# Zachary-Luk/3D-Denoising-Diffusion-Model

Measured on AMD Instinct MI355X. Metric: denoised 64³ volumes/sec @250 DDPM steps, 1/2/4/8 MI355X; PSNR vs ref, higher is better.
Workload: dtype f32 (conv products: 3x f16-split MFMA, f32 accumulate)

## Files before the change

3d-denoising-diffusion-model_amd/csrc/api.hip:

```cpp
#include <hip/hip_runtime.h>
#include <stdarg.h>
#include <stdio.h>
#include <string.h>
#include "conv3d_params.h"
#include "ddpm3d.h"
#include "ops.h"

static thread_local char g_err[512] = "";

static int fail(int code, const char* fmt, ...) {
    va_list ap;
    va_start(ap, fmt);
    vsnprintf(g_err, sizeof(g_err), fmt, ap);
    va_end(ap);
    return code;
}
static int launched(hipError_t e, const char* what) {
    if (e == hipSuccess) return DDPM3D_OK;
    return fail(DDPM3D_ELAUNCH, "%s: %s", what, hipGetErrorString(e));
}
static bool aligned16(const void* p) { return (reinterpret_cast<uintptr_t>(p) & 15) == 0; }

extern "C" {

// ... 22 lines not shown
    if (!aligned16(out)) return fail(DDPM3D_EINVAL, "pack_conv_weight: w_packed must be 16-byte aligned");
    if (prec_wz(precision) && !wz_layer_ok(Cout, Cin, ksize))
        return fail(DDPM3D_ENOSUP, "pack_conv_weight: the Winograd-D form needs ksize 3, Cout %% 128 == 0, "
                                   "Cin %% 16 == 0 (got Cout=%d Cin=%d k=%d)", Cout, Cin, ksize);
    return launched(ddpm3d_launch_pack(w, Cout, Cin, ksize, precision, out, (hipStream_t)stream),
                    "pack_conv_weight");
}

size_t ddpm3d_packed_up_phase_bytes(int Cout, int Cin) {
    if (Cout <= 0 || Cin <= 0 || !wz_layer_ok(Cout, Cin, 3)) return 0;
    return ddpm3d_up_phase_bytes(Cout, Cin);
}

int ddpm3d_pack_up_phase_weight(const float* w, int Cout, int Cin, void* out, void* stream) {
    if (!w || !out || Cout <= 0 || Cin <= 0)
        return fail(DDPM3D_EINVAL, "pack_up_phase_weight: bad arguments (Cout=%d Cin=%d)", Cout, Cin);
    if (!aligned16(out)) return fail(DDPM3D_EINVAL, "pack_up_phase_weight: w_packed must be 16-byte aligned");
    if (!wz_layer_ok(Cout, Cin, 3))
        return fail(DDPM3D_ENOSUP, "pack_up_phase_weight: needs Cout %% 128 == 0, Cin %% 16 == 0 (got Cout=%d Cin=%d)",
                    Cout, Cin);
    return launched(ddpm3d_launch_pack_up_phase(w, Cout, Cin, out, (hipStream_t)stream), "pack_up_phase_weight");
}

int ddpm3d_conv_stats_rows(int N, int D, int H, int W, int Cin, int Cout, int ksize, int precision) {
    if (N <= 0 || D <= 0 || H <= 0 || W <= 0 || Cin <= 0 || Cout <= 0 || !prec_ok(precision)) return 0;
    return ddpm3d_conv_cfg(N, D, H, W, Cin, Cout, ksize, precision).stats_rows;
}

size_t ddpm3d_conv_workspace_bytes(int N, int D, int H, int W, int Cin, int Cout, int ksize, int precision) {
    if (N <= 0 || D <= 0 || H <= 0 || W <= 0 || Cin <= 0 || Cout <= 0 || !prec_ok(precision)) return 0;
    return ddpm3d_conv_cfg(N, D, H, W, Cin, Cout, ksize, precision).workspace_bytes;
}

enum { ROUTE_GENERAL = 0, ROUTE_SKINNY = 1, ROUTE_PW = 2 };
static int conv_prepare(const ddpm3d_conv_desc* d, ConvK& k, ConvCfg& c, int& route, bool for_launch) {
    if (!d) return fail(DDPM3D_EINVAL, "conv3d: null descriptor");
    if (d->N <= 0 || d->D <= 0 || d->H <= 0 || d->W <= 0 || d->Cout <= 0 || d->Cin <= 0)
        return fail(DDPM3D_EINVAL, "conv3d: non-positive shape N=%d D=%d H=%d W=%d Cin=%d Cout=%d", d->N, d->D,
                    d->H, d->W, d->Cin, d->Cout);
    if (d->ksize != 1 && d->ksize != 3) return fail(DDPM3D_EINVAL, "conv3d: ksize %d (1 or 3)", d->ksize);
    if (!prec_ok(d->precision)) return fail(DDPM3D_ENOSUP, "conv3d: precision mode %d not implemented", d->precision);
    if (d->C0 + d->C1 != d->Cin) return fail(DDPM3D_EINVAL, "conv3d: C0+C1 != Cin");
    if (for_launch && (!d->src0 || !d->w_packed || !d->bias || !d->out)) return fail(DDPM3D_EINVAL, "conv3d: null buffer");
    if (d->in_mode == DDPM3D_IN_PLANAR2) {
        if (d->Cin != 2 || d->C0 != 1 || d->C1 != 1 || (for_launch && !d->src1) || d->aff_a)
            return fail(DDPM3D_EINVAL, "conv3d: planar2 input needs C0=C1=1, two planes, no affine");
    } else {
        if (d->in_mode < 0 || d->in_mode > DDPM3D_IN_STRIDE2) return fail(DDPM3D_EINVAL, "conv3d: in_mode %d", d->in_mode);
        if (d->in_mode == DDPM3D_IN_STRIDE2 && d->ksize != 3)
            return fail(DDPM3D_EINVAL, "conv3d: the strided input mode is the 3x3x3 Downsample conv's");
        if (d->Cin % DDPM3D_CONV_CK) return fail(DDPM3D_EINVAL, "conv3d: Cin=%d not a multiple of %d", d->Cin, DDPM3D_CONV_CK);
        if (d->C1 > 0 && (d->C0 % DDPM3D_CONV_CK || (for_launch && !d->src1)))
            return fail(DDPM3D_EINVAL, "conv3d: concat needs C0 %% %d == 0 and src1", DDPM3D_CONV_CK);
        if (!aligned16(d->src0) || (d->src1 && !aligned16(d->src1)))
            return fail(DDPM3D_EINVAL, "conv3d: sources must be 16-byte aligned");
        if (d->in_mode == DDPM3D_IN_UP && ((d->H | d->W) & 1))
            return fail(DDPM3D_EINVAL, "conv3d: upsampled input needs even H, W (got %d, %d)", d->H, d->W);
    }
    if ((d->aff_a == nullptr) != (d->aff_b == nullptr)) return fail(DDPM3D_EINVAL, "conv3d: aff_a/aff_b must come together");
    if (d->aff_a && (!aligned16(d->aff_a) || !aligned16(d->aff_b)))
        return fail(DDPM3D_EINVAL, "conv3d: affine tables must be 16-byte aligned");
    if (!aligned16(d->w_packed)) return fail(DDPM3D_EINVAL, "conv3d: w_packed must be 16-byte aligned");
    if (d->res_mode < 0 || d->res_mode > 3 || (d->res_mode != DDPM3D_RES_NONE && !d->res))
        return fail(DDPM3D_EINVAL, "conv3d: residual mode %d without / with bad buffer", d->res_mode);
    if (d->res_mode == DDPM3D_RES_UP && ((d->H | d->W) & 1))
        return fail(DDPM3D_EINVAL, "conv3d: upsampled residual needs even H, W");
    if (d->bias_stride_n < 0) return fail(DDPM3D_EINVAL, "conv3d: negative bias_stride_n");
    if (d->out_layout != DDPM3D_OUT_NDHWC && d->out_layout != DDPM3D_OUT_NCDHW)
        return fail(DDPM3D_EINVAL, "conv3d: out_layout %d", d->out_layout);

    c = ddpm3d_conv_cfg(d->N, d->D, d->H, d->W, d->Cin, d->Cout, d->ksize, d->precision);
    if (d->kernel_hint & DDPM3D_HINT_SPLITK_MASK) {
        const int s_forced = (d->kernel_hint & DDPM3D_HINT_SPLITK_MASK) >> DDPM3D_HINT_SPLITK_SHIFT;
        const int nch = ddpm3d_cin_pad(d->Cin) / DDPM3D_CONV_CK;
        if (s_forced > nch || (s_forced != c.S && c.WN != 4))
            return fail(DDPM3D_EINVAL, "conv3d: a forced split factor needs Cout > 64 and S <= Cin / 16");
        ddpm3d_conv_cfg_split(c, s_forced, d->N, d->D, d->H, d->W, d->Cout);
    }
    if (prec_wz(d->precision) &&
        !(wz_layer_ok(d->Cout, d->Cin, d->ksize) && c.WN == 4 && c.MT == 4 &&
          (d->in_mode == DDPM3D_IN_SAME || d->in_mode == DDPM3D_IN_UP)))
        return fail(DDPM3D_ENOSUP, "conv3d: the Winograd-D form needs ksize 3, Cout %% 128 == 0 "
                                   "and input mode SAME or UP; use the F16X3 packing for this call");
    if (for_launch && c.S > 1 && (!d->workspace || d->workspace_bytes < c.workspace_bytes || !aligned16(d->workspace)))
        return fail(DDPM3D_EINVAL, "conv3d: this shape is split %d-way over Cin and needs %zu bytes of "
                                   "16-byte aligned workspace (got %zu)", c.S, c.workspace_bytes,
                    d->workspace ? d->workspace_bytes : (size_t)0);
    memset(&k, 0, sizeof(k));
    k.src0 = d->src0; k.src1 = d->src1; k.affA = d->aff_a; k.affB = d->aff_b;
    k.w = (const float*)d->w_packed; k.bias = d->bias; k.res = d->res; k.out = d->out; k.stats = d->stats;
    k.N = d->N; k.D = d->D; k.H = d->H; k.W = d->W; k.Cin = d->Cin; k.Cout = d->Cout;
    k.C0 = d->C0; k.C1 = d->C1;
    k.CinPad = ddpm3d_cin_pad(d->Cin); k.CoutPad = ddpm3d_cout_pad(d->Cout);
    k.in_mode = d->in_mode; k.act = d->act; k.bias_stride_n = d->bias_stride_n;
    k.res_mode = d->res_mode; k.out_layout = d->out_layout;
    k.tilesZ = c.tilesZ; k.tilesY = c.tilesY; k.tilesX = c.tilesX;
    k.stats_rows = c.stats_rows;
    k.reduce_vox = c.reduce_vox;
    k.hint = d->kernel_hint;
    bool phase = false;
    if (d->kernel_hint & DDPM3D_HINT_UP_PHASE) {
        if (d->precision != DDPM3D_PREC_F16X3_WZ || d->in_mode != DDPM3D_IN_UP)
            return fail(DDPM3D_EINVAL, "conv3d: DDPM3D_HINT_UP_PHASE needs precision F16X3_WZ and in_mode UP");
        UpPhaseGeom g;
// ... 29 lines not shown
        const long long vox = (long long)d->N * d->D * Hs * Ws;
        const long long b0 = vox * d->C0 * ((d->io_dtype & DDPM3D_IO_SRC0_BF16) ? 2 : 4);
        const long long b1 = vox * d->C1 * ((d->io_dtype & DDPM3D_IO_SRC1_BF16) ? 2 : 4);
        const size_t wb = phase ? ddpm3d_up_phase_body_bytes(d->Cout, d->Cin)
                                : ddpm3d_packed_bytes(d->Cout, d->Cin, d->ksize, d->precision);
        if (b0 >= 0xFFFFFFF0LL || b1 >= 0xFFFFFFF0LL || wb >= 0xFFFFFFF0ULL)
            return fail(DDPM3D_E2BIG, "conv3d: a source tensor or the weights exceed 4 GiB; split the batch");
        if ((long long)d->D * d->H * d->W * d->Cout * 4 >= 0xFFFFFFF0LL)
            return fail(DDPM3D_E2BIG, "conv3d: one output sample exceeds 4 GiB; tile the volume");
        k.src0_bytes = (unsigned)b0; k.src1_bytes = (unsigned)b1; k.w_bytes = (unsigned)wb;
        k.wstat = (d->kernel_hint & DDPM3D_HINT_WSTAT_ON)    ? 1
                  : (d->kernel_hint & DDPM3D_HINT_WSTAT_OFF) ? 0
                                                             : ((long long)wb > b0 + b1 ? 1 : 0);
    }
    if (phase)
        k.wscale = (const float*)((const char*)k.w + ddpm3d_up_phase_body_bytes(d->Cout, d->Cin));
    else if (c.PREC != DDPM3D_PREC_F32)
        k.wscale = (const float*)((const char*)d->w_packed +
                                  ddpm3d_packed_bytes(d->Cout, d->Cin, d->ksize, d->precision) -
                                  (size_t)ddpm3d_cout_pad(d->Cout) * 4);
    if (d->stats && d->stats_rows != k.stats_rows)
        return fail(DDPM3D_EINVAL, "conv3d: stats_rows=%d, this shape writes %d", d->stats_rows, k.stats_rows);
    if (d->stats && !aligned16(d->stats)) return fail(DDPM3D_EINVAL, "conv3d: stats must be 16-byte aligned");
    if (d->stats && d->out_layout != DDPM3D_OUT_NDHWC)
        return fail(DDPM3D_EINVAL, "conv3d: statistics only with NDHWC output");
    const long long blocks = (long long)k.N * k.tilesZ * k.tilesY * k.tilesX;
    if (blocks > 0x7fffffffLL) return fail(DDPM3D_EINVAL, "conv3d: grid too large");
    if (d->ksize == 3 && d->Cout <= 2 && d->in_mode == DDPM3D_IN_SAME && d->C1 == 0 && !d->stats &&
        d->res_mode == DDPM3D_RES_NONE &&
        ddpm3d_skinny_ok(k.CinPad, d->precision, !(d->io_dtype & DDPM3D_IO_SRC0_BF16) ? 0
                                                  : ((d->io_dtype & DDPM3D_IO_HALF_IS_F16) ? 2 : 1)))
        route = ROUTE_SKINNY;
    else
        route = ddpm3d_pw_ok(k, c, d->ksize) ? ROUTE_PW : ROUTE_GENERAL;
    return DDPM3D_OK;
}

int ddpm3d_conv3d(const ddpm3d_conv_desc* d, void* stream) {
    ConvK k;
    ConvCfg c;
    int route = ROUTE_GENERAL;
    const int ok = conv_prepare(d, k, c, route, true);
    if (ok != DDPM3D_OK) return ok;
    if (route == ROUTE_SKINNY)
        return launched(ddpm3d_launch_conv_skinny(k, d->precision, (hipStream_t)stream), "conv3d (skinny)");
    const int rc = route == ROUTE_PW ? launched(ddpm3d_launch_conv_pw(k, c, (hipStream_t)stream), "conv3d (1x1)")
                                     : launched(ddpm3d_launch_conv(k, c, (hipStream_t)stream), "conv3d");
    if (rc != DDPM3D_OK || c.S == 1) return rc;
    return launched(ddpm3d_launch_splitk_reduce(k, (hipStream_t)stream), "conv3d split-K reduce");
}

int ddpm3d_conv_plan(const ddpm3d_conv_desc* d, int* stats_rows, size_t* workspace_bytes, int* split) {
    ConvK k;
    ConvCfg c;
    int route = ROUTE_GENERAL;
    const int ok = conv_prepare(d, k, c, route, false);
    if (ok != DDPM3D_OK) return ok;
    if (stats_rows) *stats_rows = c.stats_rows;
    if (workspace_bytes) *workspace_bytes = c.workspace_bytes;
    if (split) *split = c.S;
    return DDPM3D_OK;
}

int ddpm3d_conv_kernel_family(const ddpm3d_conv_desc* d, char* name, int name_len) {
    if (!name || name_len <= 0) return fail(DDPM3D_EINVAL, "conv_kernel_family: no buffer");
    ConvK k;
    ConvCfg c;
    int route = ROUTE_GENERAL;
    const int ok = conv_prepare(d, k, c, route, false);
    if (ok != DDPM3D_OK) return ok;
    const int tile = 1 << c.TXL;
    int n;
    if (route == ROUTE_SKINNY) n = snprintf(name, (size_t)name_len, "conv3d_p%d_k3_skinny", d->precision);
    else if (route == ROUTE_PW) n = snprintf(name, (size_t)name_len, "conv1x1_p%d_t%d", d->precision, tile);
    else n = snprintf(name, (size_t)name_len, "conv3d_p%d_k%d_wn%d_t%d", d->precision, d->ksize, c.WN, tile);
    if (n < 0 || n >= name_len) return fail(DDPM3D_EINVAL, "conv_kernel_family: buffer of %d bytes is too short", name_len);
    return DDPM3D_OK;
}

int ddpm3d_gn_finalize(const double* stats0, int C0, int rows0, const double* stats1, int C1, int rows1,
// ... 505 lines not shown
```

3d-denoising-diffusion-model_amd/csrc/conv3d_params.h:

```cpp
#pragma once
#include <hip/hip_runtime.h>
#include <stddef.h>
#include <stdlib.h>
#include "ddpm3d.h"

#define DDPM3D_CONV_CK 16
#define DDPM3D_REDUCE_VOX 16
#define DDPM3D_X3_W_TARGET 8.0f

struct ConvK {
    const float* src0;
    const float* src1;
    const float* affA;
    const float* affB;
    const float* w;
    const float* bias;
    const float* res;
    float* out;
    double* stats;
    float* partial;
    const float* wscale;
    const float* in_bound;
    int in_bound_count, in_bound_stride;
    unsigned w_bytes, src0_bytes, src1_bytes;
    int N, D, H, W, Cin, Cout, C0, C1, CinPad, CoutPad;
    int in_mode, act, bias_stride_n, res_mode, out_layout, stats_rows;
    int tilesX, tilesY, tilesZ;
    int ksplit, chunks_per_split;
    int wstat;
    int reduce_vox;
    int hint;
    int io;
};

struct ConvCfg {
    int PREC;
    int KS;
    int WN;
    int MT;
    int TXL, TYL;
    int S;
    int tilesX, tilesY, tilesZ;
    int stats_rows;
    int reduce_vox;
    size_t workspace_bytes;
};

static inline int ddpm3d_round_up(int v, int m) { return (v + m - 1) / m * m; }
static inline int ddpm3d_cout_pad(int Cout) { return ddpm3d_round_up(Cout, 32); }
static inline int ddpm3d_cin_pad(int Cin) { return ddpm3d_round_up(Cin, DDPM3D_CONV_CK); }

static inline void ddpm3d_conv_cfg_split(ConvCfg& c, int S, int N, int D, int H, int W, int Cout) {
    const long long vox = (long long)D * H * W;
    c.S = S;
    if (S > 1) {
        c.stats_rows = (int)((vox + c.reduce_vox - 1) / c.reduce_vox);
        c.workspace_bytes = (size_t)S * N * vox * Cout * sizeof(float);
    } else {
        c.stats_rows = c.tilesZ * c.tilesY * c.tilesX * (4 / c.WN);
        c.workspace_bytes = 0;
    }
}

static inline ConvCfg ddpm3d_conv_cfg(int N, int D, int H, int W, int Cin, int Cout, int ksize, int prec) {
    ConvCfg c;
    c.PREC = prec;
    const bool one_mfma = prec == DDPM3D_PREC_F16 || prec == DDPM3D_PREC_F16_WZ || prec == DDPM3D_PREC_BF16 ||
                          prec == DDPM3D_PREC_BF16_WZ;
    c.KS = ksize;
    c.WN = Cout > 64 ? 4 : (Cout > 32 ? 2 : 1);
#ifdef DDPM3D_FORCE_T4_3X3
    if (H >= 8 && W >= 8 && ksize != 3) { c.TXL = 3; c.TYL = 3; } else { c.TXL = 2; c.TYL = 2; }
#else
    if (H >= 8 && W >= 8) { c.TXL = 3; c.TYL = 3; } else { c.TXL = 2; c.TYL = 2; }
#endif
    c.MT = c.WN;
    const int TX = 1 << c.TXL, TY = 1 << c.TYL, TZ = (4 / c.WN) * c.MT * 32 / (TX * TY);
    c.tilesX = (W + TX - 1) / TX;
    c.tilesY = (H + TY - 1) / TY;
    c.tilesZ = (D + TZ - 1) / TZ;
    const long long mtiles = (long long)N * c.tilesZ * c.tilesY * c.tilesX;
    const long long blocks = mtiles * ((ddpm3d_cout_pad(Cout) + 32 * c.WN - 1) / (32 * c.WN));
    const int nch = ddpm3d_cin_pad(Cin) / DDPM3D_CONV_CK;
    int best = 1;
    if (ksize == 1 && c.WN == 4) {
        double best_cost = 1e300;
        for (int s = 1; s <= 32 && s <= nch; ++s) {
            const int cps = (nch + s - 1) / s;
            if (s > 1 && cps < 4) break;
            const long long per_cu = (blocks * s + 255) / 256;
            const double cost = (double)per_cu * (0.25 * cps + 6.0) + (s > 1 ? 6.0 : 0.0);
            if (cost < best_cost * 0.9) { best_cost = cost; best = s; }
        }
    }
    if (ksize == 3 && c.WN == 4 && !one_mfma) {
        static const double eff[4] = {1.0, 0.62, 0.78, 0.82};
        double best_cost = 1e300;
        for (int s = 1; s <= 16 && s <= nch; ++s) {
            const int cps = (nch + s - 1) / s;
            if (s > 1 && cps < 2) break;
            const long long per_cu = (blocks * s + 255) / 256;
            const double e = eff[per_cu > 3 ? 3 : (int)per_cu];
            const double cost = (double)per_cu * (cps + (s > 1 ? 0.75 : 0.5)) / e;
            if (cost < best_cost * 0.99) { best_cost = cost; best = s; }
        }
    }
    if (ksize == 3 && c.WN == 4 && one_mfma) {
        static const double eff[4] = {1.0, 0.5, 1.0, 0.9};
        static const int cand[] = {1, 2, 3, 4, 5, 6, 8, 10, 12, 16};
        const double out_mb = (double)N * D * H * W * Cout * 4.0 / 1e6;
        double best_cost = 1e300;
        for (int i = 0; i < 10 && cand[i] <= nch; ++i) {
            const int s = cand[i];
            const int cps = (nch + s - 1) / s;
            if (s > 1 && cps < 2) break;
            const long long per_cu = (blocks * s + 255) / 256;
            const double e = eff[per_cu > 3 ? 3 : (int)per_cu];
            const double cost = (double)per_cu * (cps + (s > 1 ? 3.0 : 0.25)) / e + (s > 1 ? 0.2 * s * out_mb : 0.0);
// ... 32 lines not shown
    const int TZ = 128 / (g.TX * g.TY);
    g.tilesX = (Wl + g.TX - 1) / g.TX;
    g.tilesY = (Hl + g.TY - 1) / g.TY;
    g.tilesZ = (D + TZ - 1) / TZ;
    return 4LL * g.tilesX * g.tilesY * g.tilesZ == (long long)c.tilesX * c.tilesY * c.tilesZ;
}

struct DynLdsOnce { unsigned long long mask[4]; };
static inline hipError_t ddpm3d_allow_dynamic_lds(DynLdsOnce& done, const void* kernel, int bytes) {
    int dev = 0;
    hipError_t e = hipGetDevice(&dev);
    if (e != hipSuccess) return e;
    dev &= 255;
    unsigned long long& w = done.mask[dev >> 6];
    const unsigned long long bit = 1ull << (dev & 63);
    if (__atomic_load_n(&w, __ATOMIC_ACQUIRE) & bit) return hipSuccess;
    e = hipFuncSetAttribute(kernel, hipFuncAttributeMaxDynamicSharedMemorySize, bytes);
    if (e == hipSuccess) __atomic_fetch_or(&w, bit, __ATOMIC_RELEASE);
    return e;
}

hipError_t ddpm3d_launch_conv(const ConvK& k, const ConvCfg& c, hipStream_t st);
hipError_t ddpm3d_launch_splitk_reduce(const ConvK& k, hipStream_t st);
hipError_t ddpm3d_launch_conv_skinny(const ConvK& k, int prec, hipStream_t st);
hipError_t ddpm3d_launch_conv_pw(const ConvK& k, const ConvCfg& c, hipStream_t st);
static inline bool ddpm3d_pw_ok(const ConvK& k, const ConvCfg& c, int ksize) {
    const bool s0 = (k.io & DDPM3D_IO_SRC0_BF16) != 0, s1 = (k.io & DDPM3D_IO_SRC1_BF16) != 0;
    return ksize == 1 && (c.PREC == 1 || c.PREC == 2 || c.PREC == 5) && c.WN == 4 && c.MT == 4 &&
           k.in_mode == DDPM3D_IN_SAME && k.affA == nullptr && k.act == 0 && k.stats == nullptr &&
           k.Cout % 128 == 0 && k.Cin % 32 == 0 && k.C0 % 32 == 0 && (k.C1 == 0 || s0 == s1) &&
           (k.ksplit == 1 || k.chunks_per_split % 2 == 0);
}
bool ddpm3d_skinny_ok(int CinPad, int prec, int src16);

struct GnAcc {
#ifdef DDPM3D_STATS_F64
    double a1, a2;
    __device__ __forceinline__ void init(float) { a1 = 0.0; a2 = 0.0; }
    __device__ __forceinline__ void add(float v) { const double d = (double)v; a1 += d; a2 = __builtin_fma(d, d, a2); }
    __device__ __forceinline__ double sum1(float) const { return a1; }
    __device__ __forceinline__ double sum2(float) const { return a2; }
#else
    float p, s1, s2;
    __device__ __forceinline__ void init(float pivot) { p = pivot; s1 = 0.0f; s2 = 0.0f; }
    __device__ __forceinline__ void add(float v) { const float d = v - p; s1 += d; s2 = __builtin_fmaf(d, d, s2); }
    __device__ __forceinline__ double sum1(float n) const { return (double)n * (double)p + (double)s1; }
    __device__ __forceinline__ double sum2(float n) const {
        const double dp = (double)p;
        return (double)s2 + 2.0 * dp * (double)s1 + (double)n * dp * dp;
    }
#endif
};

__device__ __forceinline__ float ddpm3d_half_to_float(unsigned short h, bool f16) {
    if (f16) return (float)__builtin_bit_cast(_Float16, h);
    return __builtin_bit_cast(float, (unsigned)h << 16);
}
__device__ __forceinline__ float ddpm3d_act_load(const float* base, size_t e, bool b16, bool f16) {
    if (b16) return ddpm3d_half_to_float(reinterpret_cast<const unsigned short*>(base)[e], f16);
    return base[e];
}
__device__ __forceinline__ unsigned short ddpm3d_to_bf16(float v) {
    return __builtin_bit_cast(unsigned short, (__bf16)v);
}
__device__ __forceinline__ unsigned short ddpm3d_to_half(float v, bool f16) {
    if (f16) return __builtin_bit_cast(unsigned short, (_Float16)v);
// ... 30 lines not shown
```

3d-denoising-diffusion-model_amd/guided_diffusion/_hip.py:

```python

import ctypes as C
import os

import torch

_HERE = os.path.dirname(os.path.abspath(__file__))
LIB_PATH = os.environ.get("DDPM3D_LIB") or os.path.normpath(os.path.join(_HERE, "..", "csrc", "libddpm3d.so"))

IN_SAME, IN_POOL, IN_UP, IN_PLANAR2, IN_STRIDE2 = 0, 1, 2, 3, 4
RES_NONE, RES_SAME, RES_POOL, RES_UP = 0, 1, 2, 3
ACT_NONE, ACT_SILU = 0, 1
OUT_NDHWC, OUT_NCDHW = 0, 1
F_LEARN_SIGMA, F_PREDICT_XSTART, F_CLIP = 1, 2, 4
NCOEF = 8
NQCOEF = 4
NSCOEF = 8
S_CX, S_W0, S_W1, S_W2, S_CZ = 0, 1, 2, 3, 4
PREC_F32, PREC_F16X3, PREC_F16, PREC_F16X3_WZ, PREC_F16_WZ, PREC_BF16, PREC_BF16_WZ = 0, 1, 2, 3, 4, 5, 6
PRECISIONS = {"f32": PREC_F32, "f16x3": PREC_F16X3, "f16": PREC_F16, "bf16": PREC_BF16}
WINOGRAD_OF = {PREC_F16X3: PREC_F16X3_WZ, PREC_F16: PREC_F16_WZ, PREC_BF16: PREC_BF16_WZ}
IO_SRC0_BF16, IO_SRC1_BF16, IO_OUT_BF16, IO_RES_BF16 = 1, 2, 4, 8
IO_HALF_IS_F16 = 16
ABI_VERSION = 13
MAX_DRAWS = 64
HINT_WSTAT_OFF, HINT_WSTAT_ON = 0x100, 0x200
HINT_SPLITK_SHIFT = 16
HINT_WZ_ORDER_SHIFT = 12
HINT_UP_PHASE = 0x400
WZ_UP_PHASE_IMAGE = 0x100

_fp = C.c_void_p


class ConvDesc(C.Structure):
    _fields_ = [
        ("N", C.c_int32), ("D", C.c_int32), ("H", C.c_int32), ("W", C.c_int32),
        ("Cin", C.c_int32), ("Cout", C.c_int32), ("ksize", C.c_int32), ("in_mode", C.c_int32),
        ("src0", _fp), ("src1", _fp), ("C0", C.c_int32), ("C1", C.c_int32),
        ("aff_a", _fp), ("aff_b", _fp), ("act", C.c_int32), ("precision", C.c_int32),
        ("w_packed", _fp), ("bias", _fp), ("bias_stride_n", C.c_int32), ("res_mode", C.c_int32),
        ("res", _fp), ("out", _fp), ("out_layout", C.c_int32), ("stats_rows", C.c_int32),
        ("stats", _fp), ("workspace", _fp), ("workspace_bytes", C.c_size_t),
        ("kernel_hint", C.c_int32), ("in_bound_count", C.c_int32), ("in_bound", _fp),
        ("in_bound_stride", C.c_int32), ("io_dtype", C.c_int32),
    ]


class ConvWeights(C.Structure):
    _fields_ = [("w_packed", _fp), ("w_packed_wz", _fp), ("bias", _fp), ("Cout", C.c_int32), ("Cin", C.c_int32),
                ("ksize", C.c_int32), ("precision", C.c_int32), ("precision_wz", C.c_int32)]


class Layer(C.Structure):
    _fields_ = [("kind", C.c_int32), ("updown", C.c_int32), ("heads", C.c_int32), ("film_off", C.c_int32),
                ("norm1_gamma", _fp), ("norm1_beta", _fp), ("norm2_gamma", _fp), ("norm2_beta", _fp),
                ("conv1", ConvWeights), ("conv2", ConvWeights), ("skip", ConvWeights)]


class UnetDesc(C.Structure):
    _fields_ = [("n_layers", C.c_int32), ("layers", C.POINTER(Layer)),
                ("n_input_blocks", C.c_int32), ("input_block_layers", C.POINTER(C.c_int32)),
# ... 163 lines not shown
```

include/ddpm3d.h:

```cpp
#ifndef DDPM3D_H
#define DDPM3D_H

#include <stddef.h>
#include <stdint.h>

#ifdef __cplusplus
extern "C" {
#endif

#define DDPM3D_ABI_VERSION 13

enum {
    DDPM3D_OK = 0,
    DDPM3D_EINVAL = -1,
    DDPM3D_ELAUNCH = -2,
    DDPM3D_ENOSUP = -3,
    DDPM3D_E2BIG = -4
};

enum {
    DDPM3D_IN_SAME = 0,
    DDPM3D_IN_POOL = 1,
    DDPM3D_IN_UP = 2,
    DDPM3D_IN_PLANAR2 = 3,
// ... 26 lines not shown
    const void* w_packed;
    const float* bias;
    int32_t bias_stride_n;
    int32_t res_mode;
    const float* res;
    float* out;
    int32_t out_layout;
    int32_t stats_rows;
    double* stats;
    void* workspace;
    size_t workspace_bytes;
    int32_t kernel_hint;
    int32_t in_bound_count;
    const float* in_bound;
    int32_t in_bound_stride;
    int32_t io_dtype;
} ddpm3d_conv_desc;

enum {
    DDPM3D_IO_SRC0_BF16 = 1,
    DDPM3D_IO_SRC1_BF16 = 2,
    DDPM3D_IO_OUT_BF16 = 4,
    DDPM3D_IO_RES_BF16 = 8,
    DDPM3D_IO_HALF_IS_F16 = 16
};

enum {
    DDPM3D_HINT_WSTAT_OFF = 0x100,
    DDPM3D_HINT_WSTAT_ON = 0x200,
    DDPM3D_HINT_WZ_ORDER_SHIFT = 12,
    DDPM3D_HINT_WZ_ORDER_MASK = 0x7000,
    DDPM3D_HINT_SPLITK_SHIFT = 16,
    DDPM3D_HINT_SPLITK_MASK = 0x3F0000,
    DDPM3D_HINT_UP_PHASE = 0x400
};

#define DDPM3D_WZ_UP_PHASE_IMAGE 0x100

int ddpm3d_abi_version(void);
const char* ddpm3d_last_error(void);

enum {
    DDPM3D_PREC_F32 = 0,
    DDPM3D_PREC_F16X3 = 1,
    DDPM3D_PREC_F16 = 2,
    DDPM3D_PREC_F16X3_WZ = 3,
    DDPM3D_PREC_F16_WZ = 4,
    DDPM3D_PREC_BF16 = 5,
    DDPM3D_PREC_BF16_WZ = 6
};

size_t ddpm3d_packed_weight_bytes(int Cout, int Cin, int ksize, int precision);
int ddpm3d_pack_conv_weight(const float* w_oidhw, int Cout, int Cin, int ksize, int precision,
                            void* w_packed, void* stream);
size_t ddpm3d_packed_up_phase_bytes(int Cout, int Cin);
int ddpm3d_pack_up_phase_weight(const float* w_oidhw, int Cout, int Cin, void* w_packed, void* stream);

int ddpm3d_conv_stats_rows(int N, int D, int H, int W, int Cin, int Cout, int ksize, int precision);
size_t ddpm3d_conv_workspace_bytes(int N, int D, int H, int W, int Cin, int Cout, int ksize, int precision);
int ddpm3d_conv3d(const ddpm3d_conv_desc* desc, void* stream);
int ddpm3d_conv_kernel_family(const ddpm3d_conv_desc* desc, char* name, int name_len);
int ddpm3d_conv_plan(const ddpm3d_conv_desc* desc, int* stats_rows, size_t* workspace_bytes, int* split);

typedef struct ddpm3d_conv_weights {
    const void* w_packed;
    const void* w_packed_wz;
    const float* bias;
// ... 230 lines not shown
```

3d-denoising-diffusion-model_amd/csrc/conv1x1.hip:

```cpp
#include <hip/hip_runtime.h>
#include <type_traits>
#include "conv3d_load.h"
#include "conv3d_epilogue.h"

namespace {

#ifndef DDPM3D_PW_DEPTH_X3
#define DDPM3D_PW_DEPTH_X3 2
#endif
#ifndef DDPM3D_PW_DEPTH_ONE
#define DDPM3D_PW_DEPTH_ONE 4
#endif
#ifndef DDPM3D_PW_WGS
#define DDPM3D_PW_WGS 2
#endif
#ifndef DDPM3D_PW_WIDE
#define DDPM3D_PW_WIDE 1
#endif
constexpr int pw_depth(int prec) { return prec == 1 ? DDPM3D_PW_DEPTH_X3 : DDPM3D_PW_DEPTH_ONE; }

template <int I, int N, class F>
__device__ __forceinline__ void pw_static_for(F&& f) {
    if constexpr (I < N) {
        f(std::integral_constant<int, I>{});
// ... 156 lines not shown
#endif
        }
    }
    PW_STAMP(3);

    const int tile_in_n = (tz_i * p.tilesY + ty_i) * p.tilesX + tx_i;
    float ws[4], bs[4];
#pragma unroll
    for (int j = 0; j < 4; ++j) {
        const int cout = wg.cy * 128 + j * 32 + (lane & 31);
        const bool cv = cout < p.Cout;
        ws[j] = cv ? p.wscale[cout] : 1.0f;
        bs[j] = (cv && p.ksplit == 1) ? p.bias[(size_t)n * p.bias_stride_n + cout] : 0.0f;
    }
    if constexpr (WIDE) {
        f32x16 accs[4];
#pragma unroll
        for (int j = 0; j < 4; ++j) accs[j] = acc[j][0];
        if (conv_epilogue_lean<PREC, 4, 1, 4, TXL, TYL, false, false>(p, accs, n, z0, y0, x0, tile_in_n, wave,
                                                                     wg.cy * 128 + (lane & 31), g, wg.split, asc.inv, ws, bs)) {
            PW_STAMP(4);
            PW_DUMP();
            return;
        }
    }
#pragma unroll
    for (int j = 0; j < 4; ++j)
        conv_epilogue<PREC, 4, 1, TXL, TYL, WIDE>(p, acc[j], n, z0, y0, x0, tile_in_n, wave,
                                                  wg.cy * 128 + j * 32 + (lane & 31), g, wg.split, asc.inv, true, ws[j], bs[j]);
    PW_STAMP(4);
    PW_DUMP();
}

template <int PREC, int S16, int TXL, int TYL>
hipError_t pw_launch(const ConvK& k, hipStream_t st) {
    constexpr int NP = PREC == 1 ? 2 : 1;
    const int gx = k.N * k.tilesZ * k.tilesY * k.tilesX, gy = k.CoutPad / 128;
    hipLaunchKernelGGL((conv3d_pw_kernel<PREC, S16, TXL, TYL, DDPM3D_PW_WIDE != 0>), dim3(gx, gy, k.ksplit), dim3(256),
                       pw_depth(PREC) * 512 * NP * 16, st, k);
    return hipGetLastError();
}

template <int PREC>
hipError_t pw_launch_prec(const ConvK& k, const ConvCfg& c, hipStream_t st) {
    const bool s16 = (k.io & DDPM3D_IO_SRC0_BF16) != 0;
    if (c.TXL == 3) return s16 ? pw_launch<PREC, 1, 3, 3>(k, st) : pw_launch<PREC, 0, 3, 3>(k, st);
    return s16 ? pw_launch<PREC, 1, 2, 2>(k, st) : pw_launch<PREC, 0, 2, 2>(k, st);
}

}

hipError_t ddpm3d_launch_conv_pw(const ConvK& k, const ConvCfg& c, hipStream_t st) {
    switch (c.PREC) {
        case 1: return pw_launch_prec<1>(k, c, st);
        case 2: return pw_launch_prec<2>(k, c, st);
        case 5: return pw_launch_prec<5>(k, c, st);
    }
    return hipErrorInvalidValue;
}
```

Before: 0.3370.

## Add specialized packed-tap kernel for the first planar2 3x3x3 conv

Adds a dedicated kernel for the network's first convolution (two input planes, f16x3 precision). It packs all 27 taps times 2 channels into the MFMA K dimension, holding the weights in registers and the input halo in LDS, so that a Cin=2 problem is not padded to 16 channels per tap. The route is on by default and can be disabled with an env var or a hint. The cost is extra code paths and tight shape constraints, and it only touches one layer out of the whole UNet.

```diff
diff --git a/3d-denoising-diffusion-model_amd/csrc/api.hip b/3d-denoising-diffusion-model_amd/csrc/api.hip
--- a/3d-denoising-diffusion-model_amd/csrc/api.hip
+++ b/3d-denoising-diffusion-model_amd/csrc/api.hip
@@ -78,7 +78,14 @@
     return ddpm3d_conv_cfg(N, D, H, W, Cin, Cout, ksize, precision).workspace_bytes;
 }
 
-enum { ROUTE_GENERAL = 0, ROUTE_SKINNY = 1, ROUTE_PW = 2 };
+enum { ROUTE_GENERAL = 0, ROUTE_SKINNY = 1, ROUTE_PW = 2, ROUTE_FIRST = 3 };
+static bool first_packed_enabled() {
+    static const bool on = [] {
+        const char* e = getenv("DDPM3D_FIRST_PACKED");
+        return !(e && e[0] == '0' && e[1] == '\0');
+    }();
+    return on;
+}
 static int conv_prepare(const ddpm3d_conv_desc* d, ConvK& k, ConvCfg& c, int& route, bool for_launch) {
     if (!d) return fail(DDPM3D_EINVAL, "conv3d: null descriptor");
     if (d->N <= 0 || d->D <= 0 || d->H <= 0 || d->W <= 0 || d->Cout <= 0 || d->Cin <= 0)
@@ -211,7 +218,8 @@
                                                   : ((d->io_dtype & DDPM3D_IO_HALF_IS_F16) ? 2 : 1)))
         route = ROUTE_SKINNY;
     else
-        route = ddpm3d_pw_ok(k, c, d->ksize) ? ROUTE_PW : ROUTE_GENERAL;
+        route = ddpm3d_pw_ok(k, c, d->ksize) ? ROUTE_PW
+                : (ddpm3d_first_ok(k, c, d->ksize) && first_packed_enabled()) ? ROUTE_FIRST : ROUTE_GENERAL;
     return DDPM3D_OK;
 }
 
@@ -224,7 +232,8 @@
     if (route == ROUTE_SKINNY)
         return launched(ddpm3d_launch_conv_skinny(k, d->precision, (hipStream_t)stream), "conv3d (skinny)");
     const int rc = route == ROUTE_PW ? launched(ddpm3d_launch_conv_pw(k, c, (hipStream_t)stream), "conv3d (1x1)")
-                                     : launched(ddpm3d_launch_conv(k, c, (hipStream_t)stream), "conv3d");
+                   : route == ROUTE_FIRST ? launched(ddpm3d_launch_conv_first(k, c, (hipStream_t)stream), "conv3d (first)")
+                                          : launched(ddpm3d_launch_conv(k, c, (hipStream_t)stream), "conv3d");
     if (rc != DDPM3D_OK || c.S == 1) return rc;
     return launched(ddpm3d_launch_splitk_reduce(k, (hipStream_t)stream), "conv3d split-K reduce");
 }
diff --git a/3d-denoising-diffusion-model_amd/csrc/conv3d_first.hip b/3d-denoising-diffusion-model_amd/csrc/conv3d_first.hip
--- /dev/null
+++ b/3d-denoising-diffusion-model_amd/csrc/conv3d_first.hip
@@ -0,0 +1,143 @@
+#include <hip/hip_runtime.h>
+#include "conv3d_load.h"
+#include "conv3d_epilogue.h"
+#include "conv3d_stage.h"
+
+namespace {
+
+constexpr int F_HX = 10, F_HY = 10, F_HZ = 4, F_HV = F_HX * F_HY * F_HZ;
+constexpr int F_VB = 8;
+constexpr int F_ZERO = F_HV * F_VB;
+constexpr int F_TSPAN = (F_HY * F_HX + 4 * F_HX) * F_VB;
+constexpr int F_LDS = F_ZERO + F_TSPAN + F_VB;
+
+__host__ __device__ __forceinline__ constexpr int first_tap_off(int tap) {
+    return tap < 27 ? ((tap / 9 * F_HY + tap / 3 % 3) * F_HX + tap % 3) * F_VB : -1;
+}
+__host__ __device__ __forceinline__ constexpr int first_tile_off(int t) { return ((t >> 1) * F_HY * F_HX + (t & 1) * 4 * F_HX) * F_VB; }
+
+template <int WN>
+__global__ __launch_bounds__(256, 3) void conv3d_first_kernel(const ConvK p) {
+    constexpr int MT = WN, WM = 4 / WN;
+    constexpr int TX = 8, TY = 8, TZ = 2;
+    __shared__ __attribute__((aligned(16))) unsigned char lds[F_LDS];
+
+    const int tid = threadIdx.x;
+    const int lane = tid & 63;
+    const int wave = __builtin_amdgcn_readfirstlane(tid >> 6);
+    const int wm = wave / WN, wn = wave % WN;
+    const int half = lane >> 5;
+
+    const WgId wg = wg_id(p);
+    int tile = wg.tile;
+    const int tx_i = tile % p.tilesX; tile /= p.tilesX;
+    const int ty_i = tile % p.tilesY; tile /= p.tilesY;
+    const int tz_i = tile % p.tilesZ; tile /= p.tilesZ;
+    const int n = tile;
+    const int x0 = tx_i * TX, y0 = ty_i * TY, z0 = tz_i * TZ;
+
+    float r0[2], r1[2];
+#pragma unroll
+    for (int i = 0; i < 2; ++i) {
+        const int hv = tid + i * 256;
+        const int hz = hv / (F_HY * F_HX);
+        const int rem = hv - hz * (F_HY * F_HX);
+        const int hy = rem / F_HX;
+        const int hx = rem - hy * F_HX;
+        const int z = z0 - 1 + hz, y = y0 - 1 + hy, x = x0 - 1 + hx;
+        r0[i] = 0.0f;
+        r1[i] = 0.0f;
+        if (hv < F_HV && halo_inb(p, z, y, x)) {
+            const size_t vox = (((size_t)n * p.D + z) * p.H + y) * p.W + x;
+            r0[i] = p.src0[vox];
+            r1[i] = p.src1[vox];
+        }
+    }
+    const ActScale asc = act_scale(p, n, 1.0f);
+
+    const int cout = wg.cy * (32 * WN) + wn * 32 + (lane & 31);
+    const bool wave_active = (wg.cy * (32 * WN) + wn * 32) < p.CoutPad;
+    const int cout_ld = wave_active ? cout : 0;
+    const __amdgpu_buffer_rsrc_t wrsrc = make_rsrc(p.w, p.w_bytes);
+    const unsigned wpart = (unsigned)p.CoutPad * 32;
+    const unsigned wtap_stride = (unsigned)(p.CinPad / DDPM3D_CONV_CK) * 2 * wpart;
+    const unsigned wlane = (unsigned)cout_ld * 32;
+    unsigned bh[4][4], bl[4][4];
+#pragma unroll
+    for (int s = 0; s < 4; ++s)
+#pragma unroll
+        for (int i = 0; i < 4; ++i) {
+            const int tap = 8 * s + 4 * half + i;
+            const unsigned voff = (s < 3 || tap < 27) ? wlane + (unsigned)tap * wtap_stride : DDPM3D_OOB_OFFSET;
+            bh[s][i] = __builtin_amdgcn_raw_buffer_load_b32(wrsrc, voff, 0, 0);
+            bl[s][i] = __builtin_amdgcn_raw_buffer_load_b32(wrsrc, voff, wpart, 0);
+        }
+
+    if (tid * F_VB < F_TSPAN + F_VB) *reinterpret_cast<u32x2*>(lds + F_ZERO + tid * F_VB) = u32x2{0u, 0u};
+#pragma unroll
+    for (int i = 0; i < 2; ++i) {
+        const int hv = tid + i * 256;
+        if (hv < F_HV) {
+            unsigned hi, lo;
+            split_pair(r0[i] * asc.s, r1[i] * asc.s, hi, lo);
+            *reinterpret_cast<u32x2*>(lds + hv * F_VB) = u32x2{hi, lo};
+        }
+    }
+    __syncthreads();
+    if (!wave_active) return;
+
+    const int l = lane & 31;
+    const int rt0 = wm * MT;
+    const int arow = (((rt0 >> 1) * F_HY + (l >> 3) + 4 * (rt0 & 1)) * F_HX + (l & 7)) * F_VB;
+    int aoff[4][4];
+#pragma unroll
+    for (int s = 0; s < 4; ++s)
+#pragma unroll
+        for (int i = 0; i < 4; ++i) {
+            constexpr int NONE = -1;
+            const int t0 = first_tap_off(8 * s + i), t1 = first_tap_off(8 * s + 4 + i);
+            const int o0 = t0 == NONE ? F_ZERO : arow + t0, o1 = t1 == NONE ? F_ZERO : arow + t1;
+            aoff[s][i] = half ? o1 : o0;
+        }
+
+    f32x16 acc[MT];
+#pragma unroll
+    for (int t = 0; t < MT; ++t)
+#pragma unroll
+        for (int i = 0; i < 16; ++i) acc[t][i] = 0.0f;
+
+#pragma unroll
+    for (int s = 0; s < 4; ++s) {
+        const h8 bhi = __builtin_bit_cast(h8, u32x4{bh[s][0], bh[s][1], bh[s][2], bh[s][3]});
+        const h8 blo = __builtin_bit_cast(h8, u32x4{bl[s][0], bl[s][1], bl[s][2], bl[s][3]});
+#pragma unroll
+        for (int t = 0; t < MT; ++t) {
+            u32x2 v[4];
+#pragma unroll
+            for (int i = 0; i < 4; ++i) v[i] = *reinterpret_cast<const u32x2*>(lds + aoff[s][i] + first_tile_off(t));
+            const h8 ahi = __builtin_bit_cast(h8, u32x4{v[0][0], v[1][0], v[2][0], v[3][0]});
+            const h8 alo = __builtin_bit_cast(h8, u32x4{v[0][1], v[1][1], v[2][1], v[3][1]});
+            acc[t] = __builtin_amdgcn_mfma_f32_32x32x16_f16(alo, bhi, acc[t], 0, 0, 0);
+            acc[t] = __builtin_amdgcn_mfma_f32_32x32x16_f16(ahi, blo, acc[t], 0, 0, 0);
+            acc[t] = __builtin_amdgcn_mfma_f32_32x32x16_f16(ahi, bhi, acc[t], 0, 0, 0);
+        }
+    }
+
+    const int tile_in_n = (tz_i * p.tilesY + ty_i) * p.tilesX + tx_i;
+    conv_epilogue<1, WM, MT, 3, 3, false>(p, acc, n, z0, y0, x0, tile_in_n, wm, cout, half, wg.split, asc.inv);
+}
+
+}
+
+hipError_t ddpm3d_launch_conv_first(const ConvK& k, const ConvCfg& c, hipStream_t st) {
+    const int gx = k.N * k.tilesZ * k.tilesY * k.tilesX;
+    const int gy = (k.CoutPad + 32 * c.WN - 1) / (32 * c.WN);
+    if (k.ksplit != 1 || c.TXL != 3 || c.TYL != 3 || c.MT != c.WN) return hipErrorInvalidValue;
+    switch (c.WN) {
+        case 4: hipLaunchKernelGGL(conv3d_first_kernel<4>, dim3(gx, gy, 1), dim3(256), 0, st, k); break;
+        case 2: hipLaunchKernelGGL(conv3d_first_kernel<2>, dim3(gx, gy, 1), dim3(256), 0, st, k); break;
+        case 1: hipLaunchKernelGGL(conv3d_first_kernel<1>, dim3(gx, gy, 1), dim3(256), 0, st, k); break;
+        default: return hipErrorInvalidValue;
+    }
+    return hipGetLastError();
+}
diff --git a/3d-denoising-diffusion-model_amd/csrc/conv3d_params.h b/3d-denoising-diffusion-model_amd/csrc/conv3d_params.h
--- a/3d-denoising-diffusion-model_amd/csrc/conv3d_params.h
+++ b/3d-denoising-diffusion-model_amd/csrc/conv3d_params.h
@@ -182,6 +182,12 @@
            (k.ksplit == 1 || k.chunks_per_split % 2 == 0);
 }
 bool ddpm3d_skinny_ok(int CinPad, int prec, int src16);
+hipError_t ddpm3d_launch_conv_first(const ConvK& k, const ConvCfg& c, hipStream_t st);
+static inline bool ddpm3d_first_ok(const ConvK& k, const ConvCfg& c, int ksize) {
+    return k.in_mode == DDPM3D_IN_PLANAR2 && ksize == 3 && c.PREC == DDPM3D_PREC_F16X3 && k.Cout % 32 == 0 &&
+           k.out_layout == DDPM3D_OUT_NDHWC && !(k.io & DDPM3D_IO_OUT_BF16) && k.ksplit == 1 && c.TXL == 3 &&
+           c.TYL == 3 && k.H % 8 == 0 && k.W % 8 == 0 && k.D % 2 == 0 && !(k.hint & DDPM3D_HINT_FIRST_GENERAL);
+}
 
 struct GnAcc {
 #ifdef DDPM3D_STATS_F64
diff --git a/3d-denoising-diffusion-model_amd/guided_diffusion/_hip.py b/3d-denoising-diffusion-model_amd/guided_diffusion/_hip.py
--- a/3d-denoising-diffusion-model_amd/guided_diffusion/_hip.py
+++ b/3d-denoising-diffusion-model_amd/guided_diffusion/_hip.py
@@ -27,6 +27,7 @@
 HINT_SPLITK_SHIFT = 16
 HINT_WZ_ORDER_SHIFT = 12
 HINT_UP_PHASE = 0x400
+HINT_FIRST_GENERAL = 0x800
 WZ_UP_PHASE_IMAGE = 0x100
 
 _fp = C.c_void_p
diff --git a/include/ddpm3d.h b/include/ddpm3d.h
--- a/include/ddpm3d.h
+++ b/include/ddpm3d.h
@@ -82,7 +82,8 @@
     DDPM3D_HINT_WZ_ORDER_MASK = 0x7000,
     DDPM3D_HINT_SPLITK_SHIFT = 16,
     DDPM3D_HINT_SPLITK_MASK = 0x3F0000,
-    DDPM3D_HINT_UP_PHASE = 0x400
+    DDPM3D_HINT_UP_PHASE = 0x400,
+    DDPM3D_HINT_FIRST_GENERAL = 0x800
 };
 
 #define DDPM3D_WZ_UP_PHASE_IMAGE 0x100
```

Result: no change. 0.3379 (median of 6 runs) (+0.3%).

## Add intra-workgroup split-K 1x1 conv kernel with LDS reduction for small grids

Applied to the files above, without the earlier changes.

Adds a pointwise conv kernel that splits the Cin reduction across the four waves of a workgroup, each wave covering all four output column groups for one quarter of the tile, then sums the partial accumulators through LDS before the epilogue. It is selected by default for F16X3 1x1 layers with few blocks (up to 128), replacing the global split-K path and its separate reduce launch for those shapes. New hint bits allow forcing it on or off. The trade-off is 64KB of LDS per workgroup and a barrier-plus-LDS reduction, which may limit occupancy.

```diff
diff --git a/3d-denoising-diffusion-model_amd/csrc/api.hip b/3d-denoising-diffusion-model_amd/csrc/api.hip
--- a/3d-denoising-diffusion-model_amd/csrc/api.hip
+++ b/3d-denoising-diffusion-model_amd/csrc/api.hip
@@ -115,7 +115,10 @@
     if (d->out_layout != DDPM3D_OUT_NDHWC && d->out_layout != DDPM3D_OUT_NCDHW)
         return fail(DDPM3D_EINVAL, "conv3d: out_layout %d", d->out_layout);
 
-    c = ddpm3d_conv_cfg(d->N, d->D, d->H, d->W, d->Cin, d->Cout, d->ksize, d->precision);
+    const int pw_form = (d->kernel_hint & (DDPM3D_HINT_SPLITK_MASK | DDPM3D_HINT_PWSPLIT_OFF)) ? 1
+                        : (d->kernel_hint & DDPM3D_HINT_PWSPLIT_ON)                             ? 2
+                                                                                                : 0;
+    c = ddpm3d_conv_cfg(d->N, d->D, d->H, d->W, d->Cin, d->Cout, d->ksize, d->precision, pw_form);
     if (d->kernel_hint & DDPM3D_HINT_SPLITK_MASK) {
         const int s_forced = (d->kernel_hint & DDPM3D_HINT_SPLITK_MASK) >> DDPM3D_HINT_SPLITK_SHIFT;
         const int nch = ddpm3d_cin_pad(d->Cin) / DDPM3D_CONV_CK;
@@ -212,6 +215,7 @@
         route = ROUTE_SKINNY;
     else
         route = ddpm3d_pw_ok(k, c, d->ksize) ? ROUTE_PW : ROUTE_GENERAL;
+    if (route != ROUTE_PW) c.PWS = 0;
     return DDPM3D_OK;
 }
 
diff --git a/3d-denoising-diffusion-model_amd/csrc/conv1x1.hip b/3d-denoising-diffusion-model_amd/csrc/conv1x1.hip
--- a/3d-denoising-diffusion-model_amd/csrc/conv1x1.hip
+++ b/3d-denoising-diffusion-model_amd/csrc/conv1x1.hip
@@ -212,8 +212,182 @@
     PW_DUMP();
 }
 
+#ifndef DDPM3D_PWS_DEPTH_X3
+#define DDPM3D_PWS_DEPTH_X3 4
+#endif
+#ifndef DDPM3D_PWS_DEPTH_ONE
+#define DDPM3D_PWS_DEPTH_ONE 6
+#endif
+constexpr int pws_depth(int prec) { return prec == 1 ? DDPM3D_PWS_DEPTH_X3 : DDPM3D_PWS_DEPTH_ONE; }
+constexpr int PWS_LDS = 4 * 4 * 4096;
+
+template <int PREC, int S16, int TXL, int TYL, bool WIDE>
+__global__ __launch_bounds__(256, DDPM3D_PW_WGS) void conv3d_pws_kernel(const ConvK p) {
+    constexpr int TX = 1 << TXL, TY = 1 << TYL, TZ = 128 / (TX * TY);
+    constexpr bool LO = PREC == 1;
+    constexpr int NP = LO ? 2 : 1;
+    constexpr int NA = S16 ? 1 : 2;
+    constexpr int NB = 4 * NP;
+    constexpr int D = pws_depth(PREC);
+    static_assert(D % 2 == 0, "a slot keeps its step parity");
+    extern __shared__ __attribute__((aligned(16))) unsigned char lds[];
+
+    const int tid = threadIdx.x, lane = tid & 63, g = lane >> 5;
+    const int wave = __builtin_amdgcn_readfirstlane(tid >> 6);
+#ifdef DDPM3D_PW_STAMPS
+    unsigned long long pw_st[5];
+#endif
+    PW_STAMP(0);
+    const WgId wg = wg_id(p);
+    int tile = wg.tile;
+    const int q = tile & 3; tile >>= 2;
+    const int tx_i = tile % p.tilesX; tile /= p.tilesX;
+    const int ty_i = tile % p.tilesY; tile /= p.tilesY;
+    const int tz_i = tile % p.tilesZ; tile /= p.tilesZ;
+    const int n = tile;
+    const int x0 = tx_i * TX, y0 = ty_i * TY, z0 = tz_i * TZ;
+
+    const int m = q * 32 + (lane & 31);
+    const int z = z0 + (m >> (TXL + TYL)), y = y0 + ((m >> TXL) & (TY - 1)), x = x0 + (m & (TX - 1));
+    const bool inb = halo_inb(p, z, y, x);
+    constexpr unsigned ES = S16 ? 2u : 4u;
+    const unsigned vox = (unsigned)(((n * p.D + z) * p.H + y) * p.W + x);
+    const unsigned voff0 = inb ? vox * (unsigned)p.C0 * ES + g * 16 * ES : DDPM3D_OOB_OFFSET;
+    const unsigned voff1 = inb ? vox * (unsigned)p.C1 * ES + g * 16 * ES : DDPM3D_OOB_OFFSET;
+
+    const unsigned wpart = (unsigned)p.CoutPad * 32, wchunk_stride = 2 * wpart;
+    const unsigned wlane = (unsigned)g * wchunk_stride + (unsigned)(wg.cy * 128 + (lane & 31)) * 32;
+
+    float bound_raw = 0.0f;
+    if constexpr (PREC == 1 || PREC == 2) bound_raw = act_scale_load(p, n);
+    ActScale asc = {1.0f, 1.0f};
+
+    f32x16 acc[4];
+#pragma unroll
+    for (int j = 0; j < 4; ++j)
+#pragma unroll
+        for (int i = 0; i < 16; ++i) acc[j][i] = 0.0f;
+
+    const int nblk = p.CinPad / 32;
+    const int ub = 2 * ((wave * nblk) >> 2), ue = 2 * (((wave + 1) * nblk) >> 2);
+
+    u32x4 ar[D][NA], br[D][NB];
+    auto issue = [&](auto slot, const int u) {
+        constexpr int SL = decltype(slot)::value;
+        constexpr unsigned s = SL & 1;
+        const bool valid = u < ue;
+        const int c0 = (u >> 1) * 32;
+        const bool from0 = c0 < p.C0;
+        const __amdgpu_buffer_rsrc_t srsrc =
+            make_rsrc(from0 ? p.src0 : p.src1, valid ? (from0 ? p.src0_bytes : p.src1_bytes) : 0u);
+        const unsigned voff = from0 ? voff0 : voff1;
+        const unsigned soff = valid ? ((unsigned)(from0 ? c0 : c0 - p.C0) + 8 * s) * ES : 0u;
+#pragma unroll
+        for (int k = 0; k < NA; ++k) ar[SL][k] = buffer_load16(srsrc, voff, soff + 16 * k);
+        const __amdgpu_buffer_rsrc_t wr = make_rsrc(p.w, valid ? p.w_bytes : 0u);
+        const unsigned wsoff = valid ? (unsigned)(u & ~1) * wchunk_stride + 16 * s : 0u;
+#pragma unroll
+        for (int j = 0; j < 4; ++j)
+#pragma unroll
+            for (int part = 0; part < NP; ++part)
+                br[SL][j * NP + part] = buffer_load16(wr, wlane + 1024u * j, wsoff + wpart * part);
+    };
+    auto unit = [&](auto slot, const int u) {
+        constexpr int SL = decltype(slot)::value;
+        float v[8];
+        if constexpr (S16) {
+            const f32x4 q0 = half4_expand(u32x2{ar[SL][0][0], ar[SL][0][1]}, (p.io & DDPM3D_IO_HALF_IS_F16) != 0);
+            const f32x4 q1 = half4_expand(u32x2{ar[SL][0][2], ar[SL][0][3]}, (p.io & DDPM3D_IO_HALF_IS_F16) != 0);
+#pragma unroll
+            for (int i = 0; i < 4; ++i) { v[i] = q0[i]; v[4 + i] = q1[i]; }
+        } else {
+            const f32x4 q0 = __builtin_bit_cast(f32x4, ar[SL][0]), q1 = __builtin_bit_cast(f32x4, ar[SL][1]);
+#pragma unroll
+            for (int i = 0; i < 4; ++i) { v[i] = q0[i]; v[4 + i] = q1[i]; }
+        }
+        h8 ahi, alo;
+        pw_operand<PREC>(v, asc.s, ahi, alo);
+#pragma unroll
+        for (int j = 0; j < 4; ++j) {
+            const h8 bhi = __builtin_bit_cast(h8, br[SL][j * NP]);
+            if constexpr (LO) {
+                const h8 blo = __builtin_bit_cast(h8, br[SL][j * NP + 1]);
+                acc[j] = __builtin_amdgcn_mfma_f32_32x32x16_f16(alo, bhi, acc[j], 0, 0, 0);
+                acc[j] = __builtin_amdgcn_mfma_f32_32x32x16_f16(ahi, blo, acc[j], 0, 0, 0);
+                acc[j] = __builtin_amdgcn_mfma_f32_32x32x16_f16(ahi, bhi, acc[j], 0, 0, 0);
+            } else {
+                acc[j] = mfma16<PREC == 5>(ahi, bhi, acc[j]);
+            }
+        }
+        __builtin_amdgcn_sched_barrier(0);
+        issue(slot, u + D);
+        __builtin_amdgcn_sched_barrier(0);
+    };
+    if (ub < ue) {
+        pw_static_for<0, D>([&](auto u) { issue(u, ub + decltype(u)::value); });
+        if constexpr (PREC == 1 || PREC == 2) asc = act_scale_finish(bound_raw, 1.0f);
+        PW_STAMP(1);
+        for (int u = ub; u < ue; u += D) {
+            pw_static_for<0, D>([&](auto s) { unit(s, u + decltype(s)::value); });
+#ifdef DDPM3D_PW_STAMPS
+            if (u == ub) PW_STAMP(2);
+#endif
+        }
+    } else {
+        if constexpr (PREC == 1 || PREC == 2) asc = act_scale_finish(bound_raw, 1.0f);
+        PW_STAMP(1);
+        PW_STAMP(2);
+    }
+    PW_STAMP(3);
+
+    const int cout = wg.cy * 128 + wave * 32 + (lane & 31);
+    const bool cv = cout < p.Cout;
+    const float ws[1] = {cv ? p.wscale[cout] : 1.0f};
+    const float bs[1] = {cv ? p.bias[(size_t)n * p.bias_stride_n + cout] : 0.0f};
+#pragma unroll
+    for (int j = 0; j < 4; ++j)
+#pragma unroll
+        for (int r = 0; r < 4; ++r)
+            *reinterpret_cast<f32x4*>(lds + (((wave * 4 + j) * 4 + r) * 64 + lane) * 16) =
+                f32x4{acc[j][4 * r], acc[j][4 * r + 1], acc[j][4 * r + 2], acc[j][4 * r + 3]};
+    __syncthreads();
+    f32x16 sum[1];
+#pragma unroll
+    for (int r = 0; r < 4; ++r) {
+        f32x4 t = *reinterpret_cast<const f32x4*>(lds + (((0 * 4 + wave) * 4 + r) * 64 + lane) * 16);
+#pragma unroll
+        for (int w = 1; w < 4; ++w)
+            t += *reinterpret_cast<const f32x4*>(lds + (((w * 4 + wave) * 4 + r) * 64 + lane) * 16);
+#pragma unroll
+        for (int i = 0; i < 4; ++i) sum[0][4 * r + i] = t[i];
+    }
+
+    const int tile_in_n = (tz_i * p.tilesY + ty_i) * p.tilesX + tx_i;
+    if constexpr (WIDE) {
+        if (conv_epilogue_lean<PREC, 4, 1, 1, TXL, TYL, false, false>(p, sum, n, z0, y0, x0, tile_in_n, q, cout, g, 0,
+                                                                     asc.inv, ws, bs)) {
+            PW_STAMP(4);
+            PW_DUMP();
+            return;
+        }
+    }
+    conv_epilogue<PREC, 4, 1, TXL, TYL, WIDE>(p, sum, n, z0, y0, x0, tile_in_n, q, cout, g, 0, asc.inv, true, ws[0], bs[0]);
+    PW_STAMP(4);
+    PW_DUMP();
+}
+
 template <int PREC, int S16, int TXL, int TYL>
-hipError_t pw_launch(const ConvK& k, hipStream_t st) {
+hipError_t pws_launch(const ConvK& k, hipStream_t st) {
+    const long long gx = 4LL * k.N * k.tilesZ * k.tilesY * k.tilesX;
+    if (k.ksplit != 1 || gx > 0x7fffffffLL) return hipErrorInvalidValue;
+    hipLaunchKernelGGL((conv3d_pws_kernel<PREC, S16, TXL, TYL, DDPM3D_PW_WIDE != 0>), dim3((unsigned)gx, k.CoutPad / 128, 1),
+                       dim3(256), PWS_LDS, st, k);
+    return hipGetLastError();
+}
+
+template <int PREC, int S16, int TXL, int TYL>
+hipError_t pw_launch(const ConvK& k, const ConvCfg& c, hipStream_t st) {
+    if (c.PWS) return pws_launch<PREC, S16, TXL, TYL>(k, st);
     constexpr int NP = PREC == 1 ? 2 : 1;
     const int gx = k.N * k.tilesZ * k.tilesY * k.tilesX, gy = k.CoutPad / 128;
     hipLaunchKernelGGL((conv3d_pw_kernel<PREC, S16, TXL, TYL, DDPM3D_PW_WIDE != 0>), dim3(gx, gy, k.ksplit), dim3(256),
@@ -224,8 +398,8 @@
 template <int PREC>
 hipError_t pw_launch_prec(const ConvK& k, const ConvCfg& c, hipStream_t st) {
     const bool s16 = (k.io & DDPM3D_IO_SRC0_BF16) != 0;
-    if (c.TXL == 3) return s16 ? pw_launch<PREC, 1, 3, 3>(k, st) : pw_launch<PREC, 0, 3, 3>(k, st);
-    return s16 ? pw_launch<PREC, 1, 2, 2>(k, st) : pw_launch<PREC, 0, 2, 2>(k, st);
+    if (c.TXL == 3) return s16 ? pw_launch<PREC, 1, 3, 3>(k, c, st) : pw_launch<PREC, 0, 3, 3>(k, c, st);
+    return s16 ? pw_launch<PREC, 1, 2, 2>(k, c, st) : pw_launch<PREC, 0, 2, 2>(k, c, st);
 }
 
 }
diff --git a/3d-denoising-diffusion-model_amd/csrc/conv3d_params.h b/3d-denoising-diffusion-model_amd/csrc/conv3d_params.h
--- a/3d-denoising-diffusion-model_amd/csrc/conv3d_params.h
+++ b/3d-denoising-diffusion-model_amd/csrc/conv3d_params.h
@@ -40,6 +40,7 @@
     int MT;
     int TXL, TYL;
     int S;
+    int PWS;
     int tilesX, tilesY, tilesZ;
     int stats_rows;
     int reduce_vox;
@@ -62,9 +63,12 @@
     }
 }
 
-static inline ConvCfg ddpm3d_conv_cfg(int N, int D, int H, int W, int Cin, int Cout, int ksize, int prec) {
+#define DDPM3D_PWS_MAX_BLOCKS 128
+static inline ConvCfg ddpm3d_conv_cfg(int N, int D, int H, int W, int Cin, int Cout, int ksize, int prec,
+                                      int pw_form = 0) {
     ConvCfg c;
     c.PREC = prec;
+    c.PWS = 0;
     const bool one_mfma = prec == DDPM3D_PREC_F16 || prec == DDPM3D_PREC_F16_WZ || prec == DDPM3D_PREC_BF16 ||
                           prec == DDPM3D_PREC_BF16_WZ;
     c.KS = ksize;
@@ -83,7 +87,10 @@
     const long long blocks = mtiles * ((ddpm3d_cout_pad(Cout) + 32 * c.WN - 1) / (32 * c.WN));
     const int nch = ddpm3d_cin_pad(Cin) / DDPM3D_CONV_CK;
     int best = 1;
-    if (ksize == 1 && c.WN == 4) {
+    if (ksize == 1 && c.WN == 4 && pw_form != 1 && Cout % 128 == 0 && Cin % 32 == 0 && mtiles * 4 <= 0x7fffffffLL &&
+        (prec == DDPM3D_PREC_F16X3 || prec == DDPM3D_PREC_F16 || prec == DDPM3D_PREC_BF16))
+        c.PWS = pw_form == 2 || (prec == DDPM3D_PREC_F16X3 && blocks <= DDPM3D_PWS_MAX_BLOCKS);
+    if (ksize == 1 && c.WN == 4 && !c.PWS) {
         double best_cost = 1e300;
         for (int s = 1; s <= 32 && s <= nch; ++s) {
             const int cps = (nch + s - 1) / s;
diff --git a/3d-denoising-diffusion-model_amd/guided_diffusion/_hip.py b/3d-denoising-diffusion-model_amd/guided_diffusion/_hip.py
--- a/3d-denoising-diffusion-model_amd/guided_diffusion/_hip.py
+++ b/3d-denoising-diffusion-model_amd/guided_diffusion/_hip.py
@@ -27,6 +27,7 @@
 HINT_SPLITK_SHIFT = 16
 HINT_WZ_ORDER_SHIFT = 12
 HINT_UP_PHASE = 0x400
+HINT_PWSPLIT_OFF, HINT_PWSPLIT_ON = 0x400000, 0x800000
 WZ_UP_PHASE_IMAGE = 0x100
 
 _fp = C.c_void_p
diff --git a/include/ddpm3d.h b/include/ddpm3d.h
--- a/include/ddpm3d.h
+++ b/include/ddpm3d.h
@@ -82,7 +82,9 @@
     DDPM3D_HINT_WZ_ORDER_MASK = 0x7000,
     DDPM3D_HINT_SPLITK_SHIFT = 16,
     DDPM3D_HINT_SPLITK_MASK = 0x3F0000,
-    DDPM3D_HINT_UP_PHASE = 0x400
+    DDPM3D_HINT_UP_PHASE = 0x400,
+    DDPM3D_HINT_PWSPLIT_OFF = 0x400000,
+    DDPM3D_HINT_PWSPLIT_ON = 0x800000
 };
 
 #define DDPM3D_WZ_UP_PHASE_IMAGE 0x100
```

Measured after the change: 0.3198 before, 0.3210 after, median of 6. About the same (+0.4%).
